# WGLab/ContextSV

Measured on AMD Instinct MI355X. Metric: long reads scanned/s (whole-genome step: scan + depth + cluster + merge + CN + split passes), synthetic 30x ONT WGS, higher is better.
Workload: dtype u32

## Files before the change

### contextsv_amd/csrc/kernels/dbscan.hip

```cpp
#include "../common.hpp"
#include "../devutil.hpp"

namespace csv {

constexpr uint32_t NONE = 0xffffffffu;

struct IntervalMetric {
    struct Elem { uint32_t s, e; };
    const uint32_t *s, *e;
    double eps;
    __device__ __forceinline__ Elem load(uint64_t i) const { return Elem{s[i], e[i]}; }
    __device__ __forceinline__ static uint32_t key(const Elem &a) { return a.s; }
    __device__ __forceinline__ void window(const Elem &a, uint64_t &lo, uint64_t &hi) const
    {
        const int li = (int)(a.e - a.s);
        const double l = li > 0 ? (double)li : 0.0;
        const uint64_t wf = (uint64_t)(eps * l) + 2;
        const uint64_t wb = (uint64_t)(eps * l / (1.0 - eps)) + 2;
        hi = (uint64_t)a.s + wf;
        lo = (uint64_t)a.s > wb ? (uint64_t)a.s - wb : 0;
    }
    __device__ __forceinline__ bool nb(const Elem &a, const Elem &b) const { return iv_neighbor(a.s, a.e, b.s, b.e, eps); }
};

struct PointMetric {
    struct Elem { int32_t p; };
    const int32_t *p;
    double eps;
    __device__ __forceinline__ Elem load(uint64_t i) const { return Elem{p[i]}; }
    __device__ __forceinline__ static uint32_t key(const Elem &a) { return (uint32_t)a.p ^ 0x80000000u; }
    __device__ __forceinline__ void window(const Elem &a, uint64_t &lo, uint64_t &hi) const
    {
        const uint64_t w = (uint64_t)eps + 1, k = key(a);
        hi = k + w;
        lo = k > w ? k - w : 0;
    }
    __device__ __forceinline__ bool nb(const Elem &a, const Elem &b) const
    {
        return (double)abs(a.p - b.p) <= eps;
    }
};

constexpr int UF_TILE = 256;
constexpr int DB_HALO = 128;
constexpr int DB_G = 16;
constexpr int DB_THREADS = 1024;
constexpr int DB_GROUPS = DB_THREADS / DB_G;

__device__ __forceinline__ int group_sum(int v)
{
#pragma unroll
    for (int d = DB_G / 2; d > 0; d >>= 1) v += __shfl_xor(v, d, DB_G);
    return v;
}
__device__ __forceinline__ int group_max(int v)
{
#pragma unroll
    for (int d = DB_G / 2; d > 0; d >>= 1) v = max(v, __shfl_xor(v, d, DB_G));
    return v;
}
__device__ __forceinline__ int group_min(int v)
{
#pragma unroll
    for (int d = DB_G / 2; d > 0; d >>= 1) v = min(v, __shfl_xor(v, d, DB_G));
    return v;
}

template <class M>
struct Staged {
    typename M::Elem *sh;
    int64_t first;
    const M &m;
    __device__ __forceinline__ typename M::Elem operator()(uint64_t j) const
    {
        const int64_t k = (int64_t)j - first;
        return (k >= 0 && k < UF_TILE + 2 * DB_HALO) ? sh[k] : m.load(j);
    }
};
template <class M>
__device__ __forceinline__ Staged<M> stage_tile(const M &m, typename M::Elem *sh, uint64_t t0, uint64_t n)
{
    const int64_t first = (int64_t)t0 - DB_HALO;
    for (int k = threadIdx.x; k < UF_TILE + 2 * DB_HALO; k += blockDim.x) {
        const int64_t idx = first + k;
        if (idx >= 0 && (uint64_t)idx < n) sh[k] = m.load((uint64_t)idx);
    }
    __syncthreads();
    return Staged<M>{sh, first, m};
}

__device__ __forceinline__ uint32_t uf_load(uint32_t *p) { return __hip_atomic_load(p, __ATOMIC_RELAXED, __HIP_MEMORY_SCOPE_AGENT); }

__device__ __forceinline__ uint32_t uf_find(uint32_t *parent, uint32_t x)
{
    for (;;) {
        const uint32_t p = uf_load(&parent[x]);
        if (p == x) return x;
        const uint32_t gp = uf_load(&parent[p]);
        if (gp != p) __hip_atomic_store(&parent[x], gp, __ATOMIC_RELAXED, __HIP_MEMORY_SCOPE_AGENT);
        x = p;
    }
}

__device__ __forceinline__ void uf_union(uint32_t *parent, uint32_t a, uint32_t b)
{
    for (;;) {
        a = uf_find(parent, a);
        b = uf_find(parent, b);
        if (a == b) return;
        if (a > b) { const uint32_t t = a; a = b; b = t; }
        if (atomicCAS(&parent[b], b, a) == b) return;
    }
}

__device__ __forceinline__ uint32_t lds_ld(uint32_t *p) { return __hip_atomic_load(p, __ATOMIC_RELAXED, __HIP_MEMORY_SCOPE_WORKGROUP); }

__device__ __forceinline__ uint32_t lds_find(uint32_t *lpar, uint32_t x)
{
    for (;;) {
        const uint32_t p = lds_ld(&lpar[x]);
        if (p == x) return x;
        const uint32_t gp = lds_ld(&lpar[p]);
        if (gp != p) __hip_atomic_store(&lpar[x], gp, __ATOMIC_RELAXED, __HIP_MEMORY_SCOPE_WORKGROUP);
        x = p;
    }
}

template <class M>
__global__ void __launch_bounds__(DB_THREADS) db_count_union_kernel(M m, uint64_t n, uint64_t split, int min_pts_imm, const int *__restrict__ d_min_pts,
                                const uint32_t *__restrict__ oid, uint8_t *__restrict__ core, uint32_t *__restrict__ parent,
                                uint32_t *__restrict__ is_root, unsigned int *__restrict__ ticket)
{
    __shared__ typename M::Elem sh[UF_TILE + 2 * DB_HALO];
    __shared__ uint32_t lpar[UF_TILE], loid[UF_TILE];
    __shared__ uint8_t lcore[UF_TILE];
    const uint64_t t0 = (uint64_t)blockIdx.x * UF_TILE;
    if (threadIdx.x < UF_TILE) {
        const uint32_t li = threadIdx.x;
        const uint64_t i = t0 + li;
        lpar[li] = li;
        loid[li] = i < n ? (oid ? oid[i] : (uint32_t)i) : NONE;
        lcore[li] = 0;
    }
    const Staged<M> at = stage_tile(m, sh, t0, n);
    if (t0 + threadIdx.x == n) { is_root[n] = 0; *ticket = 0; }
    const int min_pts = d_min_pts ? *d_min_pts : min_pts_imm;
    const uint32_t g = threadIdx.x / DB_G, lane = threadIdx.x % DB_G;
    for (uint32_t li = g; li < UF_TILE; li += DB_GROUPS) {
        const uint64_t i = t0 + li;
        if (i >= n) break;
        const uint64_t s0 = i < split ? 0 : split, s1 = i < split ? split : n;
        const typename M::Elem mine = at(i);
        uint64_t lo, hi;
        m.window(mine, lo, hi);
        int cnt = 0;
        for (uint64_t j0 = i; j0 < s1 && (uint64_t)M::key(at(j0)) <= hi; j0 += DB_G) {
            const uint64_t j = j0 + lane;
            if (j < s1) { const typename M::Elem o = at(j); if ((uint64_t)M::key(o) <= hi) cnt += m.nb(mine, o); }
        }
        for (uint64_t b0 = i; b0 > s0 && (uint64_t)M::key(at(b0 - 1)) >= lo; b0 = b0 > DB_G ? b0 - DB_G : 0) {
            if (b0 >= (uint64_t)lane + 1 && b0 - 1 - lane >= s0) { const typename M::Elem o = at(b0 - 1 - lane); if ((uint64_t)M::key(o) >= lo) cnt += m.nb(mine, o); }
            if (b0 <= DB_G) break;
        }
        cnt = group_sum(cnt);
        if (lane == 0) {
            const uint32_t me = loid[li];
            parent[me] = me;
            is_root[me] = 0;
            core[i] = cnt >= min_pts;
            lcore[li] = cnt >= min_pts;
        }
    }
    __syncthreads();
    typename M::Elem *tile = sh + DB_HALO;
    for (uint32_t li = g; li < UF_TILE; li += DB_GROUPS) {
        if (!lcore[li]) continue;
        const uint64_t i = t0 + li;
        const typename M::Elem mine = tile[li];
        uint64_t lo, hi;
        m.window(mine, lo, hi);
        const uint64_t s1 = i < split ? split : n;
        const uint32_t l_end = (uint32_t)(min(t0 + UF_TILE, s1) - t0);
        for (uint32_t j0 = li + 1; j0 < l_end && (uint64_t)M::key(tile[j0]) <= hi; j0 += DB_G) {
            const uint32_t lj = j0 + lane;
            if (lj >= l_end) continue;
            const typename M::Elem o = tile[lj];
            if ((uint64_t)M::key(o) > hi || !lcore[lj] || !m.nb(mine, o)) continue;
            uint32_t a = li, b = lj;
            for (;;) {
                a = lds_find(lpar, a);
                b = lds_find(lpar, b);
                if (a == b) break;
                if (loid[a] > loid[b]) { const uint32_t t = a; a = b; b = t; }
                if (atomicCAS(&lpar[b], b, a) == b) break;
            }
        }
    }
    __syncthreads();
    if (threadIdx.x < UF_TILE && lcore[threadIdx.x]) parent[loid[threadIdx.x]] = loid[lds_find(lpar, threadIdx.x)];
}

template <class M>
__global__ void db_union_cross_kernel(M m, uint64_t n, uint64_t split, const uint8_t *__restrict__ core, const uint32_t *__restrict__ oid, uint32_t *parent)
{
    const uint64_t i = (uint64_t)blockIdx.x * blockDim.x + threadIdx.x;
    if (i >= n || !core[i]) return;
    const uint64_t s1 = i < split ? split : n;
    const uint64_t tile_end = (i / UF_TILE + 1) * UF_TILE;
    if (tile_end >= s1) return;
    const typename M::Elem mine = m.load(i);
    uint64_t lo, hi;
    m.window(mine, lo, hi);
    if ((uint64_t)M::key(m.load(tile_end)) > hi) return;
    const uint32_t me = oid ? oid[i] : (uint32_t)i;
    uint32_t last_parent = NONE;
    for (uint64_t j = tile_end; j < s1; j++) {
        const typename M::Elem o = m.load(j);
        if ((uint64_t)M::key(o) > hi) break;
        if (!core[j] || !m.nb(mine, o)) continue;
        const uint32_t oj = oid ? oid[j] : (uint32_t)j;
        const uint32_t pj = parent[oj];
        if (pj == last_parent) continue;
        last_parent = pj;
        uf_union(parent, me, oj);
    }
}

__global__ void __launch_bounds__(UF_TILE) db_roots_rank_kernel(uint64_t n, const uint8_t *__restrict__ core, const uint32_t *__restrict__ parent,
                                                                uint32_t *__restrict__ root_of, uint32_t *__restrict__ rank,
                                                                uint32_t *__restrict__ tile_count, uint32_t *__restrict__ tile_prefix,
                                                                unsigned int *__restrict__ ticket, uint32_t n_tiles)
{
    __shared__ uint32_t wtot[UF_TILE / 64];
    __shared__ bool last;
    const uint64_t i = (uint64_t)blockIdx.x * UF_TILE + threadIdx.x;
    bool is_root = false;
    if (i < n) {
        uint32_t r = NONE;
        if (core[i]) {
            uint32_t x = (uint32_t)i;
            for (;;) { const uint32_t p = parent[x]; if (p == x) break; x = p; }
            r = x;
            is_root = x == (uint32_t)i;
        }
        root_of[i] = r;
    }
    const uint64_t bal = __ballot(is_root);
    const int w = threadIdx.x >> 6;
    if ((threadIdx.x & 63) == 0) wtot[w] = (uint32_t)__popcll(bal);
    __syncthreads();
    uint32_t before = (uint32_t)__popcll(bal & lanemask_lt());
    uint32_t total = 0;
    for (int k = 0; k < UF_TILE / 64; k++) { if (k < w) before += wtot[k]; total += wtot[k]; }
    if (i <= n) rank[i] = before;
    if (threadIdx.x == 0) {
        tile_count[blockIdx.x] = total;
        __threadfence();
        last = atomicAdd(ticket, 1u) == gridDim.x - 1;
    }
    __syncthreads();
    if (!last) return;
    __threadfence();
    __shared__ uint32_t carry_s;
    if (threadIdx.x == 0) carry_s = 0;
    __syncthreads();
    for (uint32_t c0 = 0; c0 < n_tiles; c0 += UF_TILE) {
        const uint32_t k = c0 + threadIdx.x;
        const uint32_t v = k < n_tiles ? __hip_atomic_load(&tile_count[k], __ATOMIC_RELAXED, __HIP_MEMORY_SCOPE_AGENT) : 0u;
        const uint32_t inc = wave_incl_sum_dpp(v);
        if ((threadIdx.x & 63) == 63) wtot[w] = inc;
        __syncthreads();
        uint32_t base = carry_s;
        for (int q = 0; q < w; q++) base += wtot[q];
        if (k < n_tiles) tile_prefix[k] = base + inc - v;
        __syncthreads();
        if (threadIdx.x == UF_TILE - 1) carry_s = base + inc;
        __syncthreads();
    }
}

__global__ void db_roots_kernel(uint64_t n, const uint8_t *__restrict__ core, const uint32_t *__restrict__ oid,
                                uint32_t *parent, uint32_t *__restrict__ root_of, uint32_t *__restrict__ is_root)
{
    const uint64_t i = (uint64_t)blockIdx.x * blockDim.x + threadIdx.x;
    if (i >= n) return;
    if (!core[i]) { root_of[i] = NONE; return; }
    const uint32_t me = oid ? oid[i] : (uint32_t)i;
    uint32_t x = me;
    for (;;) { const uint32_t p = parent[x]; if (p == x) break; x = p; }
    root_of[i] = x;
    if (x == me) is_root[me] = 1;
}

struct ScanCid { const uint32_t *c; __device__ __forceinline__ uint32_t operator()(uint32_t k) const { return c[k]; } };
struct TileCid {
    const uint32_t *tile_prefix, *rank;
    __device__ __forceinline__ uint32_t operator()(uint32_t k) const { return tile_prefix[k / UF_TILE] + rank[k]; }
};

template <class M, class C>
__global__ void __launch_bounds__(DB_THREADS) db_label_kernel(M m, uint64_t n, uint64_t split, const uint32_t *__restrict__ oid, const uint32_t *__restrict__ root_of,
                                C cid_raw, int32_t *__restrict__ labels)
{
    __shared__ typename M::Elem sh[UF_TILE + 2 * DB_HALO];
    const uint64_t t0 = (uint64_t)blockIdx.x * UF_TILE;
    const Staged<M> at = stage_tile(m, sh, t0, n);
    const uint32_t g = threadIdx.x / DB_G, lane = threadIdx.x % DB_G;
    for (uint32_t li = g; li < UF_TILE; li += DB_GROUPS) {
        const uint64_t i = t0 + li;
        if (i >= n) break;
        const uint32_t me = oid ? oid[i] : (uint32_t)i;
        const uint32_t r = root_of[i];
        const uint32_t id0 = (i >= split && split < n) ? cid_raw((uint32_t)split) : 0u;
        const uint64_t s0 = i < split ? 0 : split, s1 = i < split ? split : n;
        struct { C c; uint32_t off; __device__ uint32_t operator[](uint32_t k) const { return c(k) - off; } } cid{cid_raw, id0};
        if (r != NONE) { if (lane == 0) labels[me] = (int32_t)cid[r]; continue; }
        const typename M::Elem mine = at(i);
        uint64_t lo, hi;
        m.window(mine, lo, hi);
        int32_t max_start = -1, min_core = INT32_MAX;
        auto visit = [&](uint64_t j, const typename M::Elem &o) {
            if (!m.nb(mine, o)) return;
            const uint32_t rj = root_of[j];
            if (rj == NONE) return;
            const int32_t c = (int32_t)cid[rj];
            if (rj == (oid ? oid[j] : (uint32_t)j)) max_start = max(max_start, c); else min_core = min(min_core, c);
        };
        for (uint64_t j0 = i + 1; j0 < s1 && (uint64_t)M::key(at(j0)) <= hi; j0 += DB_G) {
            const uint64_t j = j0 + lane;
            if (j < s1) { const typename M::Elem o = at(j); if ((uint64_t)M::key(o) <= hi) visit(j, o); }
        }
        for (uint64_t b0 = i; b0 > s0 && (uint64_t)M::key(at(b0 - 1)) >= lo; b0 = b0 > DB_G ? b0 - DB_G : 0) {
            if (b0 >= (uint64_t)lane + 1 && b0 - 1 - lane >= s0) { const typename M::Elem o = at(b0 - 1 - lane); if ((uint64_t)M::key(o) >= lo) visit(b0 - 1 - lane, o); }
            if (b0 <= DB_G) break;
        }
        max_start = group_max(max_start);
        min_core = group_min(min_core);
        if (lane == 0) labels[me] = max_start >= 0 ? max_start : (min_core != INT32_MAX ? min_core : -2);
    }
}

size_t dbscan_tmp_bytes(uint64_t n)
{
    const uint64_t nt = (n + UF_TILE) / UF_TILE + 1;
    return align_up(n, 256) + 2 * align_up(n * 4, 256) + align_up((n + 1) * 4, 256) + exclusive_sum_tmp_bytes(n + 1) + 2 * align_up(nt * 4, 256) + 256;
}

template <class M>
static void run_dbscan(hipStream_t s, M m, const uint32_t *oid, uint64_t n, uint64_t split, int min_pts, const int *d_min_pts,
                       int32_t *labels, void *tmp)
{
    if (n == 0) return;
    char *p = (char *)tmp;
    uint8_t *core = (uint8_t *)p;      p += align_up(n, 256);
    uint32_t *parent = (uint32_t *)p;  p += align_up(n * 4, 256);
    uint32_t *root_of = (uint32_t *)p; p += align_up(n * 4, 256);
    uint32_t *cid = (uint32_t *)p;     p += align_up((n + 1) * 4, 256);
    void *es_tmp = p;                  p += exclusive_sum_tmp_bytes(n + 1);
    const uint32_t n_tiles = (uint32_t)((n + UF_TILE) / UF_TILE);
    uint32_t *tile_count = (uint32_t *)p;  p += align_up(((uint64_t)n_tiles + 1) * 4, 256);
    uint32_t *tile_prefix = (uint32_t *)p; p += align_up(((uint64_t)n_tiles + 1) * 4, 256);
    unsigned int *ticket = (unsigned int *)p;
    const dim3 grid((unsigned)((n + 255) / 256)), grid1((unsigned)((n + 1 + 255) / 256)), blk(256);
    const dim3 wide(DB_THREADS);
    hipLaunchKernelGGL(db_count_union_kernel<M>, grid1, wide, 0, s, m, n, split, min_pts, d_min_pts, oid, core, parent, cid, ticket);
    hipLaunchKernelGGL(db_union_cross_kernel<M>, grid, blk, 0, s, m, n, split, core, oid, parent);
    if (!oid) {
        hipLaunchKernelGGL(db_roots_rank_kernel, dim3(n_tiles), dim3(UF_TILE), 0, s, n, core, parent, root_of, cid, tile_count, tile_prefix, ticket, n_tiles);
        hipLaunchKernelGGL((db_label_kernel<M, TileCid>), grid, wide, 0, s, m, n, split, oid, root_of, TileCid{tile_prefix, cid}, labels);
    } else {
        hipLaunchKernelGGL(db_roots_kernel, grid, blk, 0, s, n, core, oid, parent, root_of, cid);
        launch_exclusive_sum_u32(s, cid, n + 1, es_tmp);
        hipLaunchKernelGGL((db_label_kernel<M, ScanCid>), grid, wide, 0, s, m, n, split, oid, root_of, ScanCid{cid}, labels);
    }
}

void launch_dbscan_iv_sorted(hipStream_t s, const uint32_t *start, const uint32_t *end, const uint32_t *oid,
                             uint64_t n, uint64_t split, double eps, int min_pts, const int *d_min_pts, int32_t *labels, void *tmp)
{
    IntervalMetric m{start, end, eps};
    run_dbscan(s, m, oid, n, oid ? n : split, min_pts, d_min_pts, labels, tmp);
}

size_t dbscan1d_big_tmp_bytes(uint64_t n) { return dbscan_tmp_bytes(n); }

void launch_dbscan_1d_big(hipStream_t s, const int32_t *pts_sorted, const uint32_t *oid, uint64_t n, double eps,
                          int min_pts, int32_t *labels, void *tmp)
{
    PointMetric m{pts_sorted, eps};
    run_dbscan(s, m, oid, n, n, min_pts, nullptr, labels, tmp);
}

__device__ __forceinline__ bool ivs_nb(uint32_t s1, uint32_t e1, uint32_t s2, uint32_t e2, double eps)
{
    if (min((int)e1, (int)e2) <= max((int)s1, (int)s2)) return false;
    return iv_neighbor(s1, e1, s2, e2, eps);
}

constexpr int IVS_THREADS = 1024;
constexpr int IVS_MAX = (int)DBSCAN_IV_SMALL_MAX;

__global__ __launch_bounds__(IVS_THREADS) void dbscan_iv_small_kernel(const uint32_t *__restrict__ start, const uint32_t *__restrict__ end,
                                                                     const uint64_t *__restrict__ seg_off, uint64_t n_seg, double eps, int min_pts,
                                                                     int32_t *__restrict__ labels)
{
    __shared__ uint32_t ls[IVS_MAX], le[IVS_MAX], lpar[IVS_MAX], lcid[IVS_MAX + 1];
    __shared__ uint8_t lcore[IVS_MAX];
    __shared__ uint32_t wave_tot[IVS_THREADS / WAVE];
    for (uint64_t seg = blockIdx.x; seg < n_seg; seg += gridDim.x) {
        const uint64_t o0 = seg_off[seg];
        const uint64_t n64 = seg_off[seg + 1] - o0;
        if (n64 == 0 || n64 > (uint64_t)IVS_MAX) continue;
        const int n = (int)n64;
        __syncthreads();
        for (int i = threadIdx.x; i < n; i += IVS_THREADS) { ls[i] = start[o0 + i]; le[i] = end[o0 + i]; lpar[i] = (uint32_t)i; }
        __syncthreads();
        for (int i = threadIdx.x; i < n; i += IVS_THREADS) {
            const uint32_t si = ls[i], ei = le[i];
            int cnt = 0;
            for (int j = 0; j < n; j++) cnt += ivs_nb(si, ei, ls[j], le[j], eps);
            lcore[i] = cnt >= min_pts;
        }
        __syncthreads();
        for (int i = threadIdx.x; i < n; i += IVS_THREADS) {
            if (!lcore[i]) continue;
            const uint32_t si = ls[i], ei = le[i];
            for (int j = i + 1; j < n; j++) {
                if (!lcore[j] || !ivs_nb(si, ei, ls[j], le[j], eps)) continue;
                uint32_t a = (uint32_t)i, b = (uint32_t)j;
                for (;;) {
                    a = lds_find(lpar, a); b = lds_find(lpar, b);
                    if (a == b) break;
                    if (a > b) { const uint32_t t = a; a = b; b = t; }
                    if (atomicCAS(&lpar[b], b, a) == b) break;
                }
            }
        }
        __syncthreads();
        uint32_t carry = 0;
        for (int i0 = 0; i0 < n; i0 += IVS_THREADS) {
            const int i = i0 + (int)threadIdx.x;
            const uint32_t v = (i < n && lcore[i] && lds_ld(&lpar[i]) == (uint32_t)i) ? 1u : 0u;
            const uint32_t incl = wave_incl_sum(v);
            if (lane_id() == 63) wave_tot[threadIdx.x >> 6] = incl;
            __syncthreads();
            uint32_t before = carry;
            for (int w = 0; w < (int)(threadIdx.x >> 6); w++) before += wave_tot[w];
            if (i < n) lcid[i] = before + incl - v;
            uint32_t tot = 0;
            for (int w = 0; w < IVS_THREADS / WAVE; w++) tot += wave_tot[w];
            carry += tot;
            __syncthreads();
        }
        for (int i = threadIdx.x; i < n; i += IVS_THREADS) {
            int32_t lab;
            if (lcore[i]) {
                lab = (int32_t)lcid[lds_find(lpar, (uint32_t)i)];
            } else {
                const uint32_t si = ls[i], ei = le[i];
                int32_t max_start = -1, min_core = INT32_MAX;
                for (int j = 0; j < n; j++) {
                    if (!lcore[j] || !ivs_nb(si, ei, ls[j], le[j], eps)) continue;
                    const uint32_t rj = lds_find(lpar, (uint32_t)j);
                    const int32_t c = (int32_t)lcid[rj];
                    if (rj == (uint32_t)j) max_start = max(max_start, c); else min_core = min(min_core, c);
                }
                lab = max_start >= 0 ? max_start : (min_core != INT32_MAX ? min_core : -2);
            }
            labels[o0 + i] = lab;
        }
    }
}

__global__ __launch_bounds__(IVS_THREADS) void dbscan_iv_small_sorted_kernel(const uint32_t *__restrict__ start, const uint32_t *__restrict__ end,
                                                                            const uint64_t *__restrict__ seg_off, uint64_t n_seg, double eps, int min_pts,
                                                                            int32_t *__restrict__ labels)
{
    __shared__ uint32_t ss[IVS_MAX], se[IVS_MAX], oi[IVS_MAX];
    __shared__ uint32_t lpar[IVS_MAX], lcid[IVS_MAX + 1];
    __shared__ int32_t acc[IVS_MAX], bmin[IVS_MAX];
    __shared__ uint8_t lcore[IVS_MAX];
    __shared__ uint32_t wave_tot[IVS_THREADS / WAVE];
    for (uint64_t seg = blockIdx.x; seg < n_seg; seg += gridDim.x) {
        const uint64_t o0 = seg_off[seg];
        const uint64_t n64 = seg_off[seg + 1] - o0;
        if (n64 == 0 || n64 > (uint64_t)IVS_MAX) continue;
        const int n = (int)n64;
        int np2 = 1;
        while (np2 < n) np2 <<= 1;
        __syncthreads();
        for (int i = threadIdx.x; i < np2; i += IVS_THREADS) {
            ss[i] = i < n ? (start[o0 + i] ^ 0x80000000u) : 0xffffffffu;
            oi[i] = (uint32_t)i;
            if (i < n) { lpar[i] = (uint32_t)i; acc[i] = 0; bmin[i] = INT32_MAX; }
        }
        __syncthreads();
        for (int k = 2; k <= np2; k <<= 1)
            for (int j = k >> 1; j > 0; j >>= 1) {
                for (int t = threadIdx.x; t < np2 / 2; t += IVS_THREADS) {
                    const int lo = ((t / j) * 2 * j) + (t % j), hi = lo + j;
                    const bool up = (lo & k) == 0;
                    const uint32_t a = ss[lo], b = ss[hi], ia = oi[lo], ib = oi[hi];
                    const bool gt = a > b || (a == b && ia > ib);
                    if (gt == up) { ss[lo] = b; ss[hi] = a; oi[lo] = ib; oi[hi] = ia; }
                }
                __syncthreads();
            }
        for (int p = threadIdx.x; p < n; p += IVS_THREADS) { ss[p] ^= 0x80000000u; se[p] = end[o0 + oi[p]]; }
        __syncthreads();
        for (int p = threadIdx.x; p < n; p += IVS_THREADS) {
            const uint32_t sp = ss[p], ep = se[p];
            int c = ivs_nb(sp, ep, sp, ep, eps) ? 1 : 0;
            for (int q = p + 1; q < n && (int)ss[q] < (int)ep; q++)
                if (ivs_nb(sp, ep, ss[q], se[q], eps)) { c++; atomicAdd(&acc[oi[q]], 1); }
            atomicAdd(&acc[oi[p]], c);
        }
        __syncthreads();
        for (int i = threadIdx.x; i < n; i += IVS_THREADS) lcore[i] = acc[i] >= min_pts;
        __syncthreads();
        for (int p = threadIdx.x; p < n; p += IVS_THREADS) {
            acc[oi[p]] = -1;
            if (!lcore[oi[p]]) continue;
            const uint32_t sp = ss[p], ep = se[p];
            for (int q = p + 1; q < n && (int)ss[q] < (int)ep; q++) {
                if (!lcore[oi[q]] || !ivs_nb(sp, ep, ss[q], se[q], eps)) continue;
                uint32_t a = oi[p], b = oi[q];
                for (;;) {
                    a = lds_find(lpar, a); b = lds_find(lpar, b);
                    if (a == b) break;
                    if (a > b) { const uint32_t t = a; a = b; b = t; }
                    if (atomicCAS(&lpar[b], b, a) == b) break;
                }
            }
        }
        __syncthreads();
        uint32_t carry = 0;
        for (int i0 = 0; i0 < n; i0 += IVS_THREADS) {
            const int i = i0 + (int)threadIdx.x;
            const uint32_t v = (i < n && lcore[i] && lds_ld(&lpar[i]) == (uint32_t)i) ? 1u : 0u;
            const uint32_t incl = wave_incl_sum(v);
            if (lane_id() == 63) wave_tot[threadIdx.x >> 6] = incl;
            __syncthreads();
            uint32_t before = carry;
            for (int w = 0; w < (int)(threadIdx.x >> 6); w++) before += wave_tot[w];
            if (i < n) lcid[i] = before + incl - v;
            uint32_t tot = 0;
            for (int w = 0; w < IVS_THREADS / WAVE; w++) tot += wave_tot[w];
            carry += tot;
            __syncthreads();
        }
        for (int p = threadIdx.x; p < n; p += IVS_THREADS) {
            const uint32_t sp = ss[p], ep = se[p], a = oi[p];
            const bool ca = lcore[a];
            for (int q = p + 1; q < n && (int)ss[q] < (int)ep; q++) {
                const uint32_t b = oi[q];
                const bool cb = lcore[b];
                if (ca == cb || !ivs_nb(sp, ep, ss[q], se[q], eps)) continue;
                const uint32_t core = ca ? a : b, other = ca ? b : a;
                const uint32_t r = lds_find(lpar, core);
                const int32_t c = (int32_t)lcid[r];
                if (r == core) atomicMax(&acc[other], c); else atomicMin(&bmin[other], c);
            }
        }
        __syncthreads();
        for (int i = threadIdx.x; i < n; i += IVS_THREADS) {
            int32_t lab;
            if (lcore[i]) lab = (int32_t)lcid[lds_find(lpar, (uint32_t)i)];
            else lab = acc[i] >= 0 ? acc[i] : (bmin[i] != INT32_MAX ? bmin[i] : -2);
            labels[o0 + i] = lab;
        }
    }
}

void launch_dbscan_iv_small_batched(hipStream_t s, const uint32_t *start, const uint32_t *end, const uint64_t *seg_off, uint64_t n_seg, double eps,
                                    int min_pts, int32_t *labels, bool all_pairs)
{
    if (n_seg == 0) return;
    const unsigned grid = (unsigned)std::min<uint64_t>(n_seg, 8192);
    if (all_pairs) hipLaunchKernelGGL(dbscan_iv_small_kernel, dim3(grid), dim3(IVS_THREADS), 0, s, start, end, seg_off, n_seg, eps, min_pts, labels);
    else hipLaunchKernelGGL(dbscan_iv_small_sorted_kernel, dim3(grid), dim3(IVS_THREADS), 0, s, start, end, seg_off, n_seg, eps, min_pts, labels);
}

}
```

Measured before the change: 323.6 million.

## Make DBSCAN count-union and label kernels persistent with double-buffered tile prefetch

The count/union and label kernels become persistent: at most DB_PERSIST_CAP blocks each loop over tiles, prefetching the next tile's elements, oids and roots into registers and committing them to a second LDS buffer while the current tile is processed. Neighbour windows that lie wholly inside the staged tile plus halo are counted from LDS with int indices, and the label kernel reads roots and oids from LDS, using a non-inlined global fallback only for far windows. This is meant to cut launch and occupancy overhead and hide global-load latency, at the cost of doubled LDS use, extra synchronisation and a fixed grid cap that may underuse the GPU's compute units. It also adds optional cycle-counter phase probes that are compiled out by default.

```diff
diff --git a/contextsv_amd/csrc/kernels/dbscan.hip b/contextsv_amd/csrc/kernels/dbscan.hip
--- a/contextsv_amd/csrc/kernels/dbscan.hip
+++ b/contextsv_amd/csrc/kernels/dbscan.hip
@@ -46,6 +46,11 @@
 constexpr int DB_G = 16;
 constexpr int DB_THREADS = 1024;
 constexpr int DB_GROUPS = DB_THREADS / DB_G;
+constexpr int DB_STAGE = UF_TILE + 2 * DB_HALO;
+#ifndef DB_PERSIST_CAP
+#define DB_PERSIST_CAP 128
+#endif
+constexpr uint32_t DB_CAP = DB_PERSIST_CAP;
 
 __device__ __forceinline__ int group_sum(int v)
 {
@@ -74,19 +79,20 @@
     __device__ __forceinline__ typename M::Elem operator()(uint64_t j) const
     {
         const int64_t k = (int64_t)j - first;
-        return (k >= 0 && k < UF_TILE + 2 * DB_HALO) ? sh[k] : m.load(j);
+        return (k >= 0 && k < DB_STAGE) ? sh[k] : m.load(j);
     }
 };
+struct LocalWindow { int l0, l1; uint32_t lo, hi; };
 template <class M>
-__device__ __forceinline__ Staged<M> stage_tile(const M &m, typename M::Elem *sh, uint64_t t0, uint64_t n)
-{
-    const int64_t first = (int64_t)t0 - DB_HALO;
-    for (int k = threadIdx.x; k < UF_TILE + 2 * DB_HALO; k += blockDim.x) {
-        const int64_t idx = first + k;
-        if (idx >= 0 && (uint64_t)idx < n) sh[k] = m.load((uint64_t)idx);
-    }
-    __syncthreads();
-    return Staged<M>{sh, first, m};
+__device__ __forceinline__ bool window_staged(const typename M::Elem *sh, int64_t first, uint64_t s0, uint64_t s1, uint64_t lo, uint64_t hi, LocalWindow &w)
+{
+    const bool fwd = (uint64_t)(first + DB_STAGE) >= s1 || (uint64_t)M::key(sh[DB_STAGE - DB_G]) > hi;
+    const bool bwd = first <= (int64_t)s0 || (uint64_t)M::key(sh[DB_G - 1]) < lo;
+    w.l0 = (int)max((int64_t)s0 - first, (int64_t)0);
+    w.l1 = (int)min((int64_t)s1 - first, (int64_t)DB_STAGE);
+    w.lo = (uint32_t)lo;
+    w.hi = (uint32_t)min(hi, (uint64_t)0xffffffffu);
+    return fwd && bwd;
 }
 
 __device__ __forceinline__ uint32_t uf_load(uint32_t *p) { return __hip_atomic_load(p, __ATOMIC_RELAXED, __HIP_MEMORY_SCOPE_AGENT); }
@@ -126,78 +132,156 @@
     }
 }
 
+#ifdef DBSCAN_PHASE_PROBE
+__device__ unsigned long long g_dbscan_phase[16];
+extern "C" void csvgpu_debug_dbscan_phase(unsigned long long *out, int reset)
+{
+    if (reset) { unsigned long long z[16] = {0}; (void)hipMemcpyToSymbol(HIP_SYMBOL(g_dbscan_phase), z, sizeof z); }
+    else (void)hipMemcpyFromSymbol(out, HIP_SYMBOL(g_dbscan_phase), sizeof(unsigned long long) * 16);
+}
+#define DB_PHASE_BEGIN() unsigned long long t_prev = __builtin_readcyclecounter()
+#define DB_PHASE_MARK(i) do { if (threadIdx.x == 0) { const unsigned long long t_ = __builtin_readcyclecounter(); atomicAdd(&g_dbscan_phase[i], t_ - t_prev); t_prev = t_; } } while (0)
+#define DB_PHASE_COUNT(i, v) do { if (threadIdx.x == 0) atomicAdd(&g_dbscan_phase[i], (unsigned long long)(v)); } while (0)
+#define DB_PHASE_SYNC() __syncthreads()
+#else
+#define DB_PHASE_BEGIN() do { } while (0)
+#define DB_PHASE_MARK(i) do { } while (0)
+#define DB_PHASE_COUNT(i, v) do { } while (0)
+#define DB_PHASE_SYNC() do { } while (0)
+#endif
+
+template <class M, class At>
+__device__ __forceinline__ int window_count(const M &m, const At &at, uint64_t i, uint64_t s0, uint64_t s1, const typename M::Elem &mine,
+                                            uint64_t lo, uint64_t hi, uint32_t lane)
+{
+    int cnt = 0;
+    for (uint64_t j0 = i; j0 < s1 && (uint64_t)M::key(at(j0)) <= hi; j0 += DB_G) {
+        const uint64_t j = j0 + lane;
+        if (j < s1) { const typename M::Elem o = at(j); if ((uint64_t)M::key(o) <= hi) cnt += m.nb(mine, o); }
+    }
+    for (uint64_t b0 = i; b0 > s0 && (uint64_t)M::key(at(b0 - 1)) >= lo; b0 = b0 > DB_G ? b0 - DB_G : 0) {
+        if (b0 >= (uint64_t)lane + 1 && b0 - 1 - lane >= s0) { const typename M::Elem o = at(b0 - 1 - lane); if ((uint64_t)M::key(o) >= lo) cnt += m.nb(mine, o); }
+        if (b0 <= DB_G) break;
+    }
+    return cnt;
+}
+template <class M>
+__device__ __forceinline__ int window_count_local(const M &m, const typename M::Elem *sh, int ki, const LocalWindow &w, const typename M::Elem &mine, uint32_t lane)
+{
+    int cnt = 0;
+    for (int k0 = ki; k0 < w.l1 && M::key(sh[k0]) <= w.hi; k0 += DB_G) {
+        const int k = k0 + (int)lane;
+        if (k < w.l1) { const typename M::Elem o = sh[k]; if (M::key(o) <= w.hi) cnt += m.nb(mine, o); }
+    }
+    for (int b0 = ki; b0 > w.l0 && M::key(sh[b0 - 1]) >= w.lo; b0 -= DB_G) {
+        const int k = b0 - 1 - (int)lane;
+        if (k >= w.l0) { const typename M::Elem o = sh[k]; if (M::key(o) >= w.lo) cnt += m.nb(mine, o); }
+    }
+    return cnt;
+}
+
 template <class M>
 __global__ void __launch_bounds__(DB_THREADS) db_count_union_kernel(M m, uint64_t n, uint64_t split, int min_pts_imm, const int *__restrict__ d_min_pts,
                                 const uint32_t *__restrict__ oid, uint8_t *__restrict__ core, uint32_t *__restrict__ parent,
-                                uint32_t *__restrict__ is_root, unsigned int *__restrict__ ticket)
-{
-    __shared__ typename M::Elem sh[UF_TILE + 2 * DB_HALO];
-    __shared__ uint32_t lpar[UF_TILE], loid[UF_TILE];
-    __shared__ uint8_t lcore[UF_TILE];
-    const uint64_t t0 = (uint64_t)blockIdx.x * UF_TILE;
-    if (threadIdx.x < UF_TILE) {
-        const uint32_t li = threadIdx.x;
-        const uint64_t i = t0 + li;
-        lpar[li] = li;
-        loid[li] = i < n ? (oid ? oid[i] : (uint32_t)i) : NONE;
-        lcore[li] = 0;
-    }
-    const Staged<M> at = stage_tile(m, sh, t0, n);
-    if (t0 + threadIdx.x == n) { is_root[n] = 0; *ticket = 0; }
+                                uint32_t *__restrict__ is_root, unsigned int *__restrict__ ticket, uint32_t n_tiles)
+{
+    __shared__ typename M::Elem sh[2][DB_STAGE];
+    __shared__ uint32_t lpar[2][UF_TILE], loid[2][UF_TILE];
+    __shared__ uint8_t lcore[2][UF_TILE];
+    DB_PHASE_BEGIN();
+    if (blockIdx.x == 0 && threadIdx.x == 0) { is_root[n] = 0; *ticket = 0; }
     const int min_pts = d_min_pts ? *d_min_pts : min_pts_imm;
     const uint32_t g = threadIdx.x / DB_G, lane = threadIdx.x % DB_G;
-    for (uint32_t li = g; li < UF_TILE; li += DB_GROUPS) {
-        const uint64_t i = t0 + li;
-        if (i >= n) break;
-        const uint64_t s0 = i < split ? 0 : split, s1 = i < split ? split : n;
-        const typename M::Elem mine = at(i);
-        uint64_t lo, hi;
-        m.window(mine, lo, hi);
-        int cnt = 0;
-        for (uint64_t j0 = i; j0 < s1 && (uint64_t)M::key(at(j0)) <= hi; j0 += DB_G) {
-            const uint64_t j = j0 + lane;
-            if (j < s1) { const typename M::Elem o = at(j); if ((uint64_t)M::key(o) <= hi) cnt += m.nb(mine, o); }
-        }
-        for (uint64_t b0 = i; b0 > s0 && (uint64_t)M::key(at(b0 - 1)) >= lo; b0 = b0 > DB_G ? b0 - DB_G : 0) {
-            if (b0 >= (uint64_t)lane + 1 && b0 - 1 - lane >= s0) { const typename M::Elem o = at(b0 - 1 - lane); if ((uint64_t)M::key(o) >= lo) cnt += m.nb(mine, o); }
-            if (b0 <= DB_G) break;
-        }
-        cnt = group_sum(cnt);
-        if (lane == 0) {
-            const uint32_t me = loid[li];
-            parent[me] = me;
-            is_root[me] = 0;
-            core[i] = cnt >= min_pts;
-            lcore[li] = cnt >= min_pts;
-        }
-    }
+    typename M::Elem pe{};
+    uint32_t po = 0;
+    auto fetch = [&](uint32_t t) {
+        const uint64_t f0 = (uint64_t)t * UF_TILE;
+        if (threadIdx.x < DB_STAGE) {
+            const int64_t idx = (int64_t)f0 - DB_HALO + threadIdx.x;
+            pe = m.load((uint64_t)min(max(idx, (int64_t)0), (int64_t)n - 1));
+        }
+        if (oid && threadIdx.x < UF_TILE) po = oid[min(f0 + threadIdx.x, n - 1)];
+    };
+    auto commit = [&](int b, uint32_t t) {
+        if (threadIdx.x < DB_STAGE) sh[b][threadIdx.x] = pe;
+        if (threadIdx.x < UF_TILE) {
+            const uint64_t i = (uint64_t)t * UF_TILE + threadIdx.x;
+            lpar[b][threadIdx.x] = threadIdx.x;
+            loid[b][threadIdx.x] = i < n ? (oid ? po : (uint32_t)i) : NONE;
+            lcore[b][threadIdx.x] = 0;
+        }
+    };
+    uint32_t t = blockIdx.x;
+    fetch(t);
+    commit(0, t);
     __syncthreads();
-    typename M::Elem *tile = sh + DB_HALO;
-    for (uint32_t li = g; li < UF_TILE; li += DB_GROUPS) {
-        if (!lcore[li]) continue;
-        const uint64_t i = t0 + li;
-        const typename M::Elem mine = tile[li];
-        uint64_t lo, hi;
-        m.window(mine, lo, hi);
-        const uint64_t s1 = i < split ? split : n;
-        const uint32_t l_end = (uint32_t)(min(t0 + UF_TILE, s1) - t0);
-        for (uint32_t j0 = li + 1; j0 < l_end && (uint64_t)M::key(tile[j0]) <= hi; j0 += DB_G) {
-            const uint32_t lj = j0 + lane;
-            if (lj >= l_end) continue;
-            const typename M::Elem o = tile[lj];
-            if ((uint64_t)M::key(o) > hi || !lcore[lj] || !m.nb(mine, o)) continue;
-            uint32_t a = li, b = lj;
-            for (;;) {
-                a = lds_find(lpar, a);
-                b = lds_find(lpar, b);
-                if (a == b) break;
-                if (loid[a] > loid[b]) { const uint32_t t = a; a = b; b = t; }
-                if (atomicCAS(&lpar[b], b, a) == b) break;
+    DB_PHASE_MARK(0);
+    DB_PHASE_COUNT(4, 1);
+    uint32_t flat_at = NONE, flat_root = 0;
+    for (int cur = 0; t < n_tiles; t += gridDim.x, cur ^= 1) {
+        const uint32_t t_next = t + gridDim.x;
+        if (t_next < n_tiles) fetch(t_next);
+        if (flat_at != NONE) parent[flat_at] = flat_root;
+        const uint64_t t0 = (uint64_t)t * UF_TILE;
+        const Staged<M> at{sh[cur], (int64_t)t0 - DB_HALO, m};
+        uint32_t *const par = lpar[cur], *const ids = loid[cur];
+        uint8_t *const cr = lcore[cur];
+        for (uint32_t li = g; li < UF_TILE; li += DB_GROUPS) {
+            const uint64_t i = t0 + li;
+            if (i >= n) break;
+            const uint64_t s0 = i < split ? 0 : split, s1 = i < split ? split : n;
+            const typename M::Elem mine = at(i);
+            uint64_t lo, hi;
+            m.window(mine, lo, hi);
+            LocalWindow w;
+            int cnt = window_staged<M>(sh[cur], at.first, s0, s1, lo, hi, w) ? window_count_local(m, sh[cur], DB_HALO + (int)li, w, mine, lane)
+                                                                           : window_count(m, at, i, s0, s1, mine, lo, hi, lane);
+            cnt = group_sum(cnt);
+            if (lane == 0) {
+                const uint32_t me = ids[li];
+                parent[me] = me;
+                is_root[me] = 0;
+                core[i] = cnt >= min_pts;
+                cr[li] = cnt >= min_pts;
             }
         }
-    }
-    __syncthreads();
-    if (threadIdx.x < UF_TILE && lcore[threadIdx.x]) parent[loid[threadIdx.x]] = loid[lds_find(lpar, threadIdx.x)];
+        __syncthreads();
+        DB_PHASE_MARK(1);
+        typename M::Elem *tile = sh[cur] + DB_HALO;
+        for (uint32_t li = g; li < UF_TILE; li += DB_GROUPS) {
+            if (!cr[li]) continue;
+            const uint64_t i = t0 + li;
+            const typename M::Elem mine = tile[li];
+            uint64_t lo, hi;
+            m.window(mine, lo, hi);
+            const uint64_t s1 = i < split ? split : n;
+            const uint32_t l_end = (uint32_t)(min(t0 + UF_TILE, s1) - t0);
+            for (uint32_t j0 = li + 1; j0 < l_end && (uint64_t)M::key(tile[j0]) <= hi; j0 += DB_G) {
+                const uint32_t lj = j0 + lane;
+                if (lj >= l_end) continue;
+                const typename M::Elem o = tile[lj];
+                if ((uint64_t)M::key(o) > hi || !cr[lj] || !m.nb(mine, o)) continue;
+                uint32_t a = li, b = lj;
+                for (;;) {
+                    a = lds_find(par, a);
+                    b = lds_find(par, b);
+                    if (a == b) break;
+                    if (ids[a] > ids[b]) { const uint32_t x = a; a = b; b = x; }
+                    if (atomicCAS(&par[b], b, a) == b) break;
+                }
+            }
+        }
+        __syncthreads();
+        DB_PHASE_MARK(2);
+        flat_at = NONE;
+        if (threadIdx.x < UF_TILE && cr[threadIdx.x]) { flat_at = ids[threadIdx.x]; flat_root = ids[lds_find(par, threadIdx.x)]; }
+        DB_PHASE_MARK(3);
+        DB_PHASE_COUNT(5, 1);
+        if (t_next < n_tiles) commit(cur ^ 1, t_next);
+        __syncthreads();
+        DB_PHASE_MARK(0);
+    }
+    if (flat_at != NONE) parent[flat_at] = flat_root;
 }
 
 template <class M>
@@ -292,51 +376,137 @@
     if (x == me) is_root[me] = 1;
 }
 
-struct ScanCid { const uint32_t *c; __device__ __forceinline__ uint32_t operator()(uint32_t k) const { return c[k]; } };
+struct ScanCid {
+    const uint32_t *c;
+    __device__ __forceinline__ uint32_t operator()(uint32_t k) const { return c[k]; }
+    __device__ __forceinline__ uint2 request(uint32_t k) const { return make_uint2(c[k], 0u); }
+    __device__ __forceinline__ static uint32_t value(const uint2 &p) { return p.x; }
+};
 struct TileCid {
     const uint32_t *tile_prefix, *rank;
     __device__ __forceinline__ uint32_t operator()(uint32_t k) const { return tile_prefix[k / UF_TILE] + rank[k]; }
+    __device__ __forceinline__ uint2 request(uint32_t k) const { return make_uint2(tile_prefix[k / UF_TILE], rank[k]); }
+    __device__ __forceinline__ static uint32_t value(const uint2 &p) { return p.x + p.y; }
 };
+
+template <class M, class C>
+__device__ __noinline__ int2 label_far_window(M m, uint64_t i, uint64_t s0, uint64_t s1, uint64_t lo, uint64_t hi, const uint32_t *__restrict__ oid,
+                                              const uint32_t *__restrict__ root_of, C cid_raw, uint32_t id0, uint32_t lane)
+{
+    const typename M::Elem mine = m.load(i);
+    int32_t max_start = -1, min_core = INT32_MAX;
+    auto visit = [&](uint64_t j, const typename M::Elem &o) {
+        if (!m.nb(mine, o)) return;
+        const uint32_t rj = root_of[j];
+        if (rj == NONE) return;
+        const int32_t c = (int32_t)(cid_raw(rj) - id0);
+        if (rj == (oid ? oid[j] : (uint32_t)j)) max_start = max(max_start, c); else min_core = min(min_core, c);
+    };
+    for (uint64_t j0 = i + 1; j0 < s1 && (uint64_t)M::key(m.load(j0)) <= hi; j0 += DB_G) {
+        const uint64_t j = j0 + lane;
+        if (j < s1) { const typename M::Elem o = m.load(j); if ((uint64_t)M::key(o) <= hi) visit(j, o); }
+    }
+    for (uint64_t b0 = i; b0 > s0 && (uint64_t)M::key(m.load(b0 - 1)) >= lo; b0 = b0 > DB_G ? b0 - DB_G : 0) {
+        if (b0 >= (uint64_t)lane + 1 && b0 - 1 - lane >= s0) { const typename M::Elem o = m.load(b0 - 1 - lane); if ((uint64_t)M::key(o) >= lo) visit(b0 - 1 - lane, o); }
+        if (b0 <= DB_G) break;
+    }
+    return make_int2(max_start, min_core);
+}
 
 template <class M, class C>
 __global__ void __launch_bounds__(DB_THREADS) db_label_kernel(M m, uint64_t n, uint64_t split, const uint32_t *__restrict__ oid, const uint32_t *__restrict__ root_of,
-                                C cid_raw, int32_t *__restrict__ labels)
-{
-    __shared__ typename M::Elem sh[UF_TILE + 2 * DB_HALO];
-    const uint64_t t0 = (uint64_t)blockIdx.x * UF_TILE;
-    const Staged<M> at = stage_tile(m, sh, t0, n);
+                                C cid_raw, int32_t *__restrict__ labels, uint32_t n_tiles)
+{
+    __shared__ typename M::Elem sh[2][DB_STAGE];
+    __shared__ uint32_t lroot[2][DB_STAGE], loid[2][DB_STAGE];
+    DB_PHASE_BEGIN();
+    const uint32_t id_split = split < n ? cid_raw((uint32_t)split) : 0u;
     const uint32_t g = threadIdx.x / DB_G, lane = threadIdx.x % DB_G;
-    for (uint32_t li = g; li < UF_TILE; li += DB_GROUPS) {
-        const uint64_t i = t0 + li;
-        if (i >= n) break;
-        const uint32_t me = oid ? oid[i] : (uint32_t)i;
-        const uint32_t r = root_of[i];
-        const uint32_t id0 = (i >= split && split < n) ? cid_raw((uint32_t)split) : 0u;
-        const uint64_t s0 = i < split ? 0 : split, s1 = i < split ? split : n;
-        struct { C c; uint32_t off; __device__ uint32_t operator[](uint32_t k) const { return c(k) - off; } } cid{cid_raw, id0};
-        if (r != NONE) { if (lane == 0) labels[me] = (int32_t)cid[r]; continue; }
-        const typename M::Elem mine = at(i);
-        uint64_t lo, hi;
-        m.window(mine, lo, hi);
-        int32_t max_start = -1, min_core = INT32_MAX;
-        auto visit = [&](uint64_t j, const typename M::Elem &o) {
-            if (!m.nb(mine, o)) return;
-            const uint32_t rj = root_of[j];
-            if (rj == NONE) return;
-            const int32_t c = (int32_t)cid[rj];
-            if (rj == (oid ? oid[j] : (uint32_t)j)) max_start = max(max_start, c); else min_core = min(min_core, c);
-        };
-        for (uint64_t j0 = i + 1; j0 < s1 && (uint64_t)M::key(at(j0)) <= hi; j0 += DB_G) {
-            const uint64_t j = j0 + lane;
-            if (j < s1) { const typename M::Elem o = at(j); if ((uint64_t)M::key(o) <= hi) visit(j, o); }
-        }
-        for (uint64_t b0 = i; b0 > s0 && (uint64_t)M::key(at(b0 - 1)) >= lo; b0 = b0 > DB_G ? b0 - DB_G : 0) {
-            if (b0 >= (uint64_t)lane + 1 && b0 - 1 - lane >= s0) { const typename M::Elem o = at(b0 - 1 - lane); if ((uint64_t)M::key(o) >= lo) visit(b0 - 1 - lane, o); }
-            if (b0 <= DB_G) break;
-        }
-        max_start = group_max(max_start);
-        min_core = group_min(min_core);
-        if (lane == 0) labels[me] = max_start >= 0 ? max_start : (min_core != INT32_MAX ? min_core : -2);
+    typename M::Elem pe{};
+    uint32_t pr = NONE, po = 0;
+    auto fetch = [&](uint32_t t) {
+        if (threadIdx.x < DB_STAGE) {
+            const int64_t idx = (int64_t)t * UF_TILE - DB_HALO + threadIdx.x;
+            const uint64_t j = (uint64_t)min(max(idx, (int64_t)0), (int64_t)n - 1);
+            pe = m.load(j);
+            pr = root_of[j];
+            if (oid) po = oid[j];
+        }
+    };
+    auto commit = [&](int b, uint32_t t) {
+        if (threadIdx.x < DB_STAGE) {
+            sh[b][threadIdx.x] = pe;
+            lroot[b][threadIdx.x] = pr;
+            loid[b][threadIdx.x] = oid ? po : (uint32_t)((int64_t)t * UF_TILE - DB_HALO + threadIdx.x);
+        }
+    };
+    uint2 my_cid = make_uint2(0u, 0u);
+    auto own = [&](int b) {
+        if (threadIdx.x < UF_TILE) {
+            const uint32_t r = lroot[b][DB_HALO + threadIdx.x];
+            my_cid = cid_raw.request(r != NONE ? r : 0u);
+        }
+    };
+    uint32_t t = blockIdx.x;
+    fetch(t);
+    commit(0, t);
+    __syncthreads();
+    own(0);
+    DB_PHASE_MARK(8);
+    DB_PHASE_COUNT(12, 1);
+    for (int cur = 0; t < n_tiles; t += gridDim.x, cur ^= 1) {
+        const uint32_t t_next = t + gridDim.x;
+        if (t_next < n_tiles) fetch(t_next);
+        const uint64_t t0 = (uint64_t)t * UF_TILE;
+        const int64_t first = (int64_t)t0 - DB_HALO;
+        const Staged<M> at{sh[cur], first, m};
+        const uint32_t *const roots = lroot[cur], *const ids = loid[cur];
+        for (uint32_t li = g; li < UF_TILE; li += DB_GROUPS) {
+            const uint64_t i = t0 + li;
+            if (i >= n) break;
+            if (roots[DB_HALO + li] != NONE) continue;
+            const uint32_t me = ids[DB_HALO + li];
+            const uint32_t id0 = i >= split ? id_split : 0u;
+            const uint64_t s0 = i < split ? 0 : split, s1 = i < split ? split : n;
+            const typename M::Elem mine = at(i);
+            uint64_t lo, hi;
+            m.window(mine, lo, hi);
+            int32_t max_start = -1, min_core = INT32_MAX;
+            auto take = [&](uint32_t rj, uint32_t oj) {
+                if (rj == NONE) return;
+                const int32_t c = (int32_t)(cid_raw(rj) - id0);
+                if (rj == oj) max_start = max(max_start, c); else min_core = min(min_core, c);
+            };
+            LocalWindow w;
+            if (window_staged<M>(sh[cur], first, s0, s1, lo, hi, w)) {
+                const typename M::Elem *const el = sh[cur];
+                for (int k0 = DB_HALO + (int)li + 1; k0 < w.l1 && M::key(el[k0]) <= w.hi; k0 += DB_G) {
+                    const int k = k0 + (int)lane;
+                    if (k < w.l1) { const typename M::Elem o = el[k]; if (M::key(o) <= w.hi && m.nb(mine, o)) take(roots[k], ids[k]); }
+                }
+                for (int b0 = DB_HALO + (int)li; b0 > w.l0 && M::key(el[b0 - 1]) >= w.lo; b0 -= DB_G) {
+                    const int k = b0 - 1 - (int)lane;
+                    if (k >= w.l0) { const typename M::Elem o = el[k]; if (M::key(o) >= w.lo && m.nb(mine, o)) take(roots[k], ids[k]); }
+                }
+            } else {
+                const int2 far = label_far_window(m, i, s0, s1, lo, hi, oid, root_of, cid_raw, id0, lane);
+                max_start = far.x;
+                min_core = far.y;
+            }
+            max_start = group_max(max_start);
+            min_core = group_min(min_core);
+            if (lane == 0) labels[me] = max_start >= 0 ? max_start : (min_core != INT32_MAX ? min_core : -2);
+        }
+        DB_PHASE_SYNC();
+        DB_PHASE_MARK(9);
+        if (t_next < n_tiles) commit(cur ^ 1, t_next);
+        if (threadIdx.x < UF_TILE && t0 + threadIdx.x < n && roots[DB_HALO + threadIdx.x] != NONE)
+            labels[ids[DB_HALO + threadIdx.x]] = (int32_t)(C::value(my_cid) - (t0 + threadIdx.x >= split ? id_split : 0u));
+        DB_PHASE_MARK(10);
+        DB_PHASE_COUNT(13, 1);
+        __syncthreads();
+        if (t_next < n_tiles) own(cur ^ 1);
+        DB_PHASE_MARK(8);
     }
 }
 
@@ -361,17 +531,18 @@
     uint32_t *tile_count = (uint32_t *)p;  p += align_up(((uint64_t)n_tiles + 1) * 4, 256);
     uint32_t *tile_prefix = (uint32_t *)p; p += align_up(((uint64_t)n_tiles + 1) * 4, 256);
     unsigned int *ticket = (unsigned int *)p;
-    const dim3 grid((unsigned)((n + 255) / 256)), grid1((unsigned)((n + 1 + 255) / 256)), blk(256);
-    const dim3 wide(DB_THREADS);
-    hipLaunchKernelGGL(db_count_union_kernel<M>, grid1, wide, 0, s, m, n, split, min_pts, d_min_pts, oid, core, parent, cid, ticket);
+    const dim3 grid((unsigned)((n + 255) / 256)), blk(256);
+    const uint32_t w_tiles = (uint32_t)((n + UF_TILE - 1) / UF_TILE);
+    const dim3 wide(DB_THREADS), pgrid(std::min(w_tiles, DB_CAP));
+    hipLaunchKernelGGL(db_count_union_kernel<M>, pgrid, wide, 0, s, m, n, split, min_pts, d_min_pts, oid, core, parent, cid, ticket, w_tiles);
     hipLaunchKernelGGL(db_union_cross_kernel<M>, grid, blk, 0, s, m, n, split, core, oid, parent);
     if (!oid) {
         hipLaunchKernelGGL(db_roots_rank_kernel, dim3(n_tiles), dim3(UF_TILE), 0, s, n, core, parent, root_of, cid, tile_count, tile_prefix, ticket, n_tiles);
-        hipLaunchKernelGGL((db_label_kernel<M, TileCid>), grid, wide, 0, s, m, n, split, oid, root_of, TileCid{tile_prefix, cid}, labels);
+        hipLaunchKernelGGL((db_label_kernel<M, TileCid>), pgrid, wide, 0, s, m, n, split, oid, root_of, TileCid{tile_prefix, cid}, labels, w_tiles);
     } else {
         hipLaunchKernelGGL(db_roots_kernel, grid, blk, 0, s, n, core, oid, parent, root_of, cid);
         launch_exclusive_sum_u32(s, cid, n + 1, es_tmp);
-        hipLaunchKernelGGL((db_label_kernel<M, ScanCid>), grid, wide, 0, s, m, n, split, oid, root_of, ScanCid{cid}, labels);
+        hipLaunchKernelGGL((db_label_kernel<M, ScanCid>), pgrid, wide, 0, s, m, n, split, oid, root_of, ScanCid{cid}, labels, w_tiles);
     }
 }
 
```

Result: slower. 300.3 million (-7.2%).
